# geek-ai/MAgent

Measured on AMD Instinct MI355X. Metric: agent-steps/sec (step+obs) on battle map; bit-exact vs CPU ref, higher is better.
Workload: dtype f32; 1 GPU; battle 1000x1000, 2x400k agents, random placement (C3(i): 2x500k does not fit 996,004 cells), random actions; envs=1, parallelism=replicas x1, gather=none, rccl_ranks=1, io=device-resident (env_*_device C-ABI)

## Files before the change

### magent_amd/csrc/engine.h

```cpp
#pragma once
#include <hip/hip_runtime.h>
#include <stdint.h>

namespace magent_amd {

constexpr int MAXG = 8;
constexpr int REF_SHIFT = 27;
constexpr int REF_MASK = (1 << REF_SHIFT) - 1;
constexpr int OCC_EMPTY = -1;
constexpr int OCC_WALL = -2;
constexpr int OCC_FOOD = -3;

constexpr int PEND_NONE = 0;
constexpr int PEND_MOVE = 1 << 16;
constexpr int PEND_ATTACK = 2 << 16;
constexpr int PEND_TURN = 3 << 16;
constexpr int PEND_ARG = 0xFFFF;

constexpr int OP_KILL = 3, OP_COLLIDE = 6, OP_ATTACK = 7, OP_NULL = 11;

constexpr int RANK_INF = 0x7FFFFFFF;
constexpr unsigned MV_FAIL = 0xFFFFFFFFu, MV_OK = 0xFFFFFFFEu;
constexpr unsigned MV_SILENT = 0xFFFFFFFDu, MV_TAKEN_BIT = 0x80000000u;
__host__ __device__ inline bool mv_taken(unsigned s) { return (s >> 30) == 2u; }
// ... 18 lines not shown
        default: rx = x + ln - 1; ry = y; break;
    }
}
__host__ __device__ inline void real_to_saved(int dir, int wd, int ln, int rx, int ry, int &x, int &y) {
    switch (dir) {
        case DIR_NORTH: x = rx; y = ry; break;
        case DIR_SOUTH: x = rx - wd + 1; y = ry - ln + 1; break;
        case DIR_WEST: x = rx; y = ry - wd + 1; break;
        default: x = rx - ln + 1; y = ry; break;
    }
}

__host__ __device__ inline int ref_pack(int g, int i) { return (g << REF_SHIFT) | i; }
__host__ __device__ inline int ref_group(int r) { return r >> REF_SHIFT; }
__host__ __device__ inline int ref_index(int r) { return r & REF_MASK; }

struct TypeDev {
    float hp, damage, step_recover, kill_supply, kill_reward, dead_penalty, attack_penalty, step_reward;
    float food_supply, eat_ability;
    int attack_in_group;
    int can_absorb;
    int bw, bl;
    int n_move, n_attack;
    int n_turn;
    int move_off, attack_off;
    int attack_bit;
    int view_w, view_h;
    int view_x1, view_y1;
    int mask_off;
};
// ... 89 lines not shown
```

### magent_amd/csrc/engine_batch.hip

```cpp
#include "engine_impl.h"

namespace magent_amd {

bool Env::cycle_eligible(int n_group, float *const *view, float *const *feat, int *first_obs_out) {
    if (!device_ready) fatal("cycle called before reset");
    const int NG = (int)groups.size();
    if (n_group != NG) fatal("env_cycle_many: n_group (%d) differs from the number of groups (%d)", n_group, NG);
    return solo_ok(total_agents()) && !step_pending && !serial_calls_on && observed_groups_ok(view, feat, true, false, first_obs_out);
}

bool Env::observed_groups_ok(float *const *view, float *const *feat, bool goals_differ, bool refuse_acted, int *first_obs_out) const {
    int n_obs = 0, first_obs = -1;
    if (first_obs_out) *first_obs_out = -1;
    for (int g = 0; g < (int)groups.size(); g++) {
        if (refuse_acted && groups[g].acted) return false;
        if (!(view && view[g]) || groups[g].n == 0) continue;
        if (!feat || !feat[g] || (((uintptr_t)view[g]) & 15) || (((uintptr_t)feat[g]) & 15)) return false;
        const HostType &t = *groups[g].type, &t0 = *groups[first_obs < 0 ? g : first_obs].type;
        if (minimap_mode && (t.view.height != t0.view.height || t.view.width != t0.view.width || (goals_differ && t.can_absorb != t0.can_absorb))) return false;
        if (first_obs < 0) first_obs = g;
        n_obs++;
    }
    if (first_obs_out) *first_obs_out = first_obs;
    return n_obs <= RENDER_MULTI_MAX;
// ... 300 lines not shown
    if ((size_t)sa_tiles > asums_cap) {
        grow(arena, d_asums, asums_cap, (size_t)sa_tiles, stream);
        grow(arena, d_wpre, wpre_cap, asums_cap * (SCAN_TILE_HOST / 64), stream);
    }
    step_live_paint = live_paint_now = paint_valid;
    step_pending = true;
    map_warm = false;
    step_kind = StepKind::Pipeline; step_fused_rules = true;
    plain_steps++;
    scratch_for(Scratch::Plain);
    shuffle_buffers(total_n);
    push_rng();
    attack_round = rounds;
    if (rounds >= 4) pairs_two_steps++; else if (rounds >= 2) pairs_one_steps++;
    it.W.live_paint = live_paint_now ? 1 : 0;
    it.PW = plain_view();
    it.ptab = d_ptab; it.gtab = d_gtab; it.ttab = d_ttab;
    it.B = shuffle_bufs(); it.powtab = d_powtab;
    it.sums = d_asums; it.wpre = d_wpre;
    it.R = strike_rules(rule_args.data(), (int)rule_args.size());
    it.seq = ++step_seq;
    it.n_max = total_n;
    alive_valid = true;
    stale_events = true;
    for (auto &g : groups) g.sa_off = -1;
    it.A = ClearArgs{};
    for (int g = 0; g < NG; g++) {
        HostGroup &G = groups[g];
        if (rewards && rewards[g] && G.n > 0) { it.rewards[g] = rewards[g]; it.group_reward[g] = G.group_reward; }
        it.A.sums_off[g] = alive_off[g];
// ... 44 lines not shown
```

### magent_amd/csrc/engine_host.h

```cpp
#pragma once
#include <condition_variable>
#include <functional>
#include <map>
#include <memory>
#include <mutex>
#include <string>
#include <thread>
#include <utility>
#include <vector>

#include "engine.h"
#include "launch.h"
#include "tune.h"

namespace magent_amd {

[[noreturn]] void fatal(const char *fmt, ...);

struct MinStd {
    unsigned long long x = 1;
    void seed(unsigned long s) { x = s % 2147483647ul; if (x == 0) x = 1; }
    unsigned long long operator()() { x = (x * 16807ull) % 2147483647ull; return x; }
    void skip(unsigned n) {
        unsigned long long b = 16807ull, a = x;
// ... 220 lines not shown
    void wait_record(int seq);
    StepRecord *h_rec = nullptr;
    int step_seq = 0;
    int solo_nt_eval = 0;
    unsigned *d_hit = nullptr;
    int2 *d_mvnodes = nullptr; size_t mvnodes_cap = 0;
    void move_nodes();
    bool claim_clean = false;
    bool claim_epochs = false;
    unsigned plain_epoch = 0;
    bool hit_clean = false;
    void scratch_for(Scratch path);
    int plain_steps = 0, plain_slots = 0;
    int pairs_two_steps = 0, pairs_one_steps = 0, claim_refills = 0;
    bool plain_world = false, step_fused_rules = false, ptab_valid = false;
    PlainGroup *d_ptab = nullptr;
    int *d_alive = nullptr; size_t alive_cap = 0;
    int alive_off[MAXG] = {}, alive_n[MAXG] = {};
    bool alive_valid = false;
    bool map_scattered = false;
    long long placed_random = 0, placed_total = 0;
    bool map_warm = false;
    PlainWorld plain_view();
    void plain_arrays(HostGroup &g, size_t n, size_t cap);
    bool stale_events = false;
    RuleArgs *d_rule_args = nullptr; RuleProg *d_rule_progs = nullptr;
    void shuffle_buffers(int n_max);
    void push_rng();
    ShuffleBufs shuffle_bufs() const;
    void attack_rounds_checked(const WorldView &W);
// ... 77 lines not shown
```

### magent_amd/csrc/engine_step.hip

```cpp
#include "engine_impl.h"

namespace magent_amd {

void Env::set_action_device(int g, const int *d_act) {
    if (g < 0 || g >= (int)groups.size()) fatal("invalid group handle in set_action : %d", g);
    use_device();
    HostGroup &G = groups[g];
    bool goals_act = G.type->can_absorb && G.n > 0 && !G.acted && !serial_calls_on;
    if (goals_act) {
        enter();
        int *flag = d_counters + CTR_GOALS_ACT;
        HIP_OK(hipMemsetAsync(flag, 0, sizeof(int), stream));
        launch_any_real_action(stream, d_act, G.n, G.tdev, d_delta, flag);
        int h_flag = 0;
        read_back(&h_flag, flag, sizeof(int));
        goals_act = h_flag != 0;
        static bool told = false;
        if (goals_act && !told) {
            told = true;
            std::fprintf(stderr, "magent-amd: a group of goals (can_absorb) was given actions that move, turn or attack: such steps run the reference's "
                                 "sequential loops on one lane of the device -- exact, about a microsecond per action of the whole world (INTEGRATION.md)\n");
        }
    }
    if (G.acted || serial_calls_on || goals_act) {
// ... 289 lines not shown
    shuffle_buffers(total_n);
    push_rng();
    scratch_for(Scratch::Solo);
    assign_pending_seq(W);
    const SoloStep S = solo_step_args();
    ProfScope p(*this, "step");
    launch_step_solo(stream, W, S);
}

bool Env::single_sync_step(const WorldView &W, int total_n, bool beside) {
    const bool plain = W.plain != 0;
    step_kind = plain ? StepKind::Pipeline : StepKind::Generic;
    if (plain) plain_steps++;
    scratch_for(plain ? Scratch::Plain : Scratch::Other);
    PlainWorld PW{};
    if (plain) PW = plain_view();
    {
        const size_t caps = rank_cap + shuf_cap + sums_cap + powtab_cap;
        const bool rng_here = !rng_on_device;
        shuffle_buffers(total_n);
        push_rng();
        if (rng_here || caps != rank_cap + shuf_cap + sums_cap + powtab_cap) state_epoch++;
    }
    hipStream_t a = beside ? side_stream() : stream;
    {
        ProfScope p(*this, "attack", false, a);
        if (plain) launch_shuffle_draw(a, total_n, d_counters, shuffle_bufs(), d_powtab, step_sa_tiled);
        else launch_shuffle(a, total_n, d_counters, shuffle_bufs(), d_rank, d_hit, (size_t)width * height, d_powtab, step_sa_tiled);
        if (overlap_level == 2 && a != stream) { join_side(); a = stream; }
        attack_round = 0;
        const int pairs = opt_fixed ? opt_attack_pairs : (boost_attack > 0 ? 2 : 1);
        if (plain) { if (pairs >= 2) pairs_two_steps++; else if (pairs == 1) pairs_one_steps++; }
        if (plain) launch_plain_rank(a, W, PW, d_ptab, shuffle_bufs(), d_asums, d_wpre, seq_plan());
        else launch_attack_rank(a, W, d_gtab, d_rank, shuffle_bufs(), false, d_asums, d_wpre, seq_plan());
        for (int r = 0; r < 2 * pairs; r++) {
            const int flag = r == 2 * pairs - 1 ? CTR_OPEN_ATTACK : -1;
            if (plain) launch_plain_eval(a, W, PW, d_ptab, d_gtab, d_ttab, ++attack_round, flag, shuffle_bufs());
            else launch_attack_iter(a, W, d_gtab, d_ttab, ++attack_round, attack_kmax, flag);
        }
        if (pairs == 0) launch_set_counter(a, d_counters, CTR_OPEN_ATTACK, 1, -1);
    }
    join_side();
    if (!plain) { generic_step_tail(W); return false; }
    return plain_step_tail(W, PW);
}

bool Env::plain_step_tail(const WorldView &W, const PlainWorld &PW) {
    const bool fuse = step_fused_rules = !rules_on_host && !stale_events && fused_rules(rule_args.data(), (int)rule_args.size());
// ... 98 lines not shown
}

PlainWorld Env::plain_view() {
    PlainWorld PW{};
    for (size_t g = 0; g < groups.size(); g++) PW.g[g] = groups[g].pl;
    PW.S = plain_slots; PW.kmax = attack_kmax;
    {
        size_t total = 0;
        for (size_t g = 0; g < groups.size(); g++) { alive_off[g] = (int)total; alive_n[g] = groups[g].n; total += (size_t)(groups[g].n + 255) / 256; }
        grow(arena, d_alive, alive_cap, std::max<size_t>(total, 1), stream);
        PW.alive = d_alive;
        for (int g = 0; g < MAXG; g++) PW.alive_off[g] = g < (int)groups.size() ? alive_off[g] : 0;
    }
    PW.epoch = 62 - (int)(plain_epoch % 63u);
    PW.round_base = (int)(plain_epoch * 64u);
    if (!ptab_valid) {
        if (!d_ptab) HIP_OK(dev_malloc(arena, &d_ptab, sizeof(PlainGroup) * MAXG));
        HIP_OK(hipMemcpyAsync(d_ptab, PW.g, sizeof(PlainGroup) * MAXG, hipMemcpyHostToDevice, stream));
        ptab_valid = true;
        state_epoch++;
    }
    return PW;
}

SeqPlan Env::seq_plan() const {
    SeqPlan P{};
    for (int g = 0; g < MAXG; g++) P.off[g] = g < (int)groups.size() ? groups[g].sa_off : -1;
    return P;
}

// ... 181 lines not shown
```

### magent_amd/csrc/launch.h

```cpp
#pragma once
#include "engine.h"

namespace magent_amd {

struct FastDiv {
    unsigned mul, shift, one;
};
inline FastDiv make_fastdiv(unsigned d) {
    FastDiv f{0, 0, 0};
    if (d <= 1) { f.one = 1; return f; }
    unsigned s = 0;
    while ((1ull << s) < d) s++;
    unsigned long long m = ((1ull << 32) * ((1ull << s) - d)) / d + 1;
    f.mul = (unsigned)m;
    f.shift = s - 1;
    return f;
}

struct RenderPlan {
    int spans;
    int steps_per_span;
    int feat_blocks;
    int xcd_chunk;
    int strip_floats;
// ... 84 lines not shown
struct SeqPlan { int off[MAXG]; };
void launch_set_action(hipStream_t s, const WorldView &W, int g, const int *actions, int call_base, int *sums, int *wpre, int tile_off );
void launch_seq_assign(hipStream_t s, const WorldView &W, int g, const int *sums, const int *wpre, int tile_off, bool write_total);
void launch_attack_rank(hipStream_t s, const WorldView &W, const GroupDev *gtab, const int *rank, const ShuffleBufs &B, bool clear_hitbits, const int *sums, const int *wpre,
                        const SeqPlan &P);
void launch_attack_iter(hipStream_t s, const WorldView &W, const GroupDev *gtab, const TypeDev *ttab, int round, int kmax, int flag );
void launch_attack_apply(hipStream_t s, const WorldView &W, const GroupDev *gtab, const TypeDev *ttab, int kmax);
struct PlainGroup { int4 *rec; int *atk; unsigned *hmask; uint2 *hlist; };
struct PlainWorld {
    PlainGroup g[MAXG];
    int S, kmax;
    int *alive;
    int alive_off[MAXG];
    int epoch;
    int round_base;
};
struct StrikeRules {
    int n;
    struct One { int ga, gb, op, rule_no, n_subj; float v[4]; } r[4];
};
StrikeRules strike_rules(const RuleArgs *rules , int n_rules);
bool fused_rules(const RuleArgs *rules, int n);
bool plain_eval_lds_ok(int kmax);
void launch_shuffle_draw(hipStream_t s, int n_max, int *counters, const ShuffleBufs &B, const unsigned *powtab, bool tiled);
void launch_plain_rank(hipStream_t s, const WorldView &W, const PlainWorld &PW, const PlainGroup *ptab, const ShuffleBufs &B, const int *sums,
                       const int *wpre, const SeqPlan &P);
void launch_plain_eval(hipStream_t s, const WorldView &W, const PlainWorld &PW, const PlainGroup *ptab, const GroupDev *gtab, const TypeDev *ttab, int round, int flag,
                       const ShuffleBufs &B);
void launch_plain_tail(hipStream_t s, const WorldView &W, const PlainWorld &PW, const PlainGroup *ptab, const GroupDev *gtab, const TypeDev *ttab,
                       const RuleArgs *rules , int n_rules, StepRecord *rec , int seq);
void launch_food_iter(hipStream_t s, const WorldView &W, const GroupDev *gtab, const TypeDev *ttab, int round, int kmax, int flag);
void launch_attack_events(hipStream_t s, const WorldView &W, int4 *ev);
void launch_move_prep(hipStream_t s, const WorldView &W, const GroupDev *gtab);
void launch_movg_prep(hipStream_t s, const WorldView &W, bool starve);
void launch_turn_prep(hipStream_t s, const WorldView &W);
void launch_turn_sweep(hipStream_t s, const WorldView &W, const GroupDev *gtab, int flag);
void launch_turn_apply(hipStream_t s, const WorldView &W);
void launch_movg_sweep(hipStream_t s, const WorldView &W, const GroupDev *gtab, int flag);
void launch_movg_apply(hipStream_t s, const WorldView &W, const GroupDev *gtab);
void launch_move_apply(hipStream_t s, const WorldView &W, const GroupDev *gtab);
void launch_rule(hipStream_t s, const WorldView &W, const RuleArgs &A);
// ... 28 lines not shown
    const PlainGroup *ptab; const GroupDev *gtab; const TypeDev *ttab;
    ShuffleBufs B; const unsigned *powtab;
    int *sums, *wpre;
    SeqPlan P;
    const int *actions[MAXG]; int call_base[MAXG];
    StrikeRules R;
    StepRecord *rec; int seq;
    int n_max;
    RenderMulti M;
    ClearArgs A;
    MiniArgs Mi; int *counts;
    const int *alive_sums;
    float *rewards[MAXG]; float group_reward[MAXG];
    GroupDev *gtab_out; TypeDev *ttab_out;
    int *newn;
    int pad_[2];
};
struct PipeCtl { const StepRecord *reports_d; StepRecord *reports_h; int *ticket; int *flag_h; int flag_seq; int n_env; };
constexpr int PIPE_REPORT_BYTES = 128;
struct PipeDims { int n_env, max_n, max_total, G, slots, render_blocks, rounds, kmax, sweep, hist_cells; size_t render_lds; };
void launch_pipe_upload(hipStream_t s, const PipeItem *h_items, PipeItem *d_items, int n_env);
void launch_pipe_cycle(hipStream_t s, const PipeItem *d_items, const PipeDims &D, const PipeCtl &C);
bool render_sweep_mini_ok(const WorldView &W, const RenderArgs &R);
size_t render_sweep_lds(int VHW, int C);

#ifndef MAGENT_SCAN_ITEMS
#define MAGENT_SCAN_ITEMS 2
#endif
constexpr int SCAN_ITEMS_HOST = MAGENT_SCAN_ITEMS;
constexpr int SCAN_TILE_HOST = 256 * SCAN_ITEMS_HOST;
constexpr int ATTACK_KMAX_HOST = 32;
// ... 3 lines not shown
```

### magent_amd/csrc/plain_dev.h

```cpp
#pragma once
#include "kernels_dev.h"

namespace magent_amd {

__device__ __forceinline__ void set_action_tile_body(const WorldView &W, int g, const int *actions, int call_base, int *sums, int *wpre, int tile_off) {
    const GroupDev &G = W.grp[g];
    const TypeDev &T = W.type[g];
    const int tile0 = blockIdx.x * SCAN_TILE;
    int act[SCAN_ITEMS], xs[SCAN_ITEMS];
#pragma unroll
    for (int k = 0; k < SCAN_ITEMS; k++) {
        const int i = tile0 + k * SCAN_THREADS + threadIdx.x;
        act[k] = i < G.n ? actions[i] : 0;
        xs[k] = (i < G.n && W.large_map) ? G.x[i] : 0;
    }
    __shared__ int s_w[SCAN_WAVES];
#pragma unroll
    for (int k = 0; k < SCAN_ITEMS; k++) {
        const int i = tile0 + k * SCAN_THREADS + threadIdx.x;
        const bool attack = i < G.n && act[k] >= T.n_move + T.n_turn && act[k] < T.n_move + T.n_turn + T.n_attack;
        const int cnt = __popcll(__ballot(attack));
        if (lane_id() == 0) s_w[k * (SCAN_THREADS / 64) + (threadIdx.x >> 6)] = cnt;
        if (i < G.n) {
            const int a = act[k];
// ... 63 lines not shown
        rec->unsupported = counters[CTR_UNSUPPORTED]; rec->pack_overflow = counters[CTR_PACK_OVERFLOW];
        rec->bad_action = counters[CTR_BAD_ACTION]; rec->hit_overflow = counters[CTR_HIT_OVERFLOW];
        rec->error = 0; rec->rounds_attack = 0; rec->rounds_move = 0; rec->n_marks = 0;
        rec->open_attack = oa; rec->open_move = om;
    }
    if (!open) {
        if (tid < CTR_TRIGGER_END - CTR_TRIGGER) counters[CTR_TRIGGER + tid] = 0;
        if (tid < ROUND_SLOTS) counters[CTR_ROUND_CHANGED + tid] = 0;
        if (tid < ATT_SLOTS) counters[att_slot(tid)] = 0;
        if (tid == 0) counters[CTR_ATTACK] = 0;
    }
    if (mode == REPORT_DEVICE) { if (tid == 0) rec->seq = seq; return; }
    __threadfence_system();
    if (tid == 0) __hip_atomic_store((int *)&rec->seq, seq, __ATOMIC_RELEASE, __HIP_MEMORY_SCOPE_SYSTEM);
}
__device__ __forceinline__ void plain_rank_body(const WorldView &W, const PlainWorld &PW, const PlainGroup *ptab, const ShuffleBufs &B, const int *sums, const int *wpre, const SeqPlan &P) {
    const int A = W.counters[CTR_ATTACK];
    if ((blockIdx.x | blockIdx.y | threadIdx.x) == 0) {
        W.counters[CTR_CHANGED] = 0;
        W.counters[CTR_LAST_A] = A;
        W.counters[CTR_RNG] = (int)rng_skip((unsigned)W.counters[CTR_RNG], (unsigned)A);
    }
    const int g = blockIdx.y;
    const int i = blockIdx.x * blockDim.x + threadIdx.x;
    const GroupDev &G = W.grp[g];
    const TypeDev &T = W.type[g];
    const int n = G.n;
    if ((int)(blockIdx.x * blockDim.x) >= n) return;
    const int pend = i < n ? G.pend[i] : PEND_NONE;
    const bool att = (pend & ~PEND_ARG) == PEND_ATTACK;
    int seq = -1;
    if (A != 0 && P.off[g] >= 0) seq = attack_seq(sums, wpre, P.off[g], i, att);
    if (i >= n) return;
    const bool dead = G.dead[i];
    const int x = G.x[i], y = G.y[i];
    unsigned key = G.key[i];
    int tgt = -1, t = -1;
    if (!dead && att) {
        key = (unsigned)shuffle_chase_pos(seq >= 0 ? seq : (int)key, A, B.j, B.head, B.first, B.link);
        const int k = pend & PEND_ARG;
        const int2 d = W.delta[T.attack_off + k];
        const int tx = x + d.x, ty = y + d.y;
        if (tx >= 0 && tx < W.w && ty >= 0 && ty < W.h) {
            const int o = W.occ[ty * W.w + tx];
            if (o >= 0 && (T.attack_in_group || ref_group(o) != g)) {
                tgt = o;
                const PlainGroup TG = ptab[ref_group(o)];
                const int slot = T.attack_bit + k;
                glob(TG.hlist)[(size_t)ref_index(o) * PW.S + slot] = make_uint2(key, (unsigned)ref_pack(g, i));
                atomicOr(&glob(TG.hmask)[ref_index(o)], 1u << slot);
            }
        }
    } else if (!dead && (pend & ~PEND_ARG) == PEND_MOVE) {
        const int2 d = W.delta[T.move_off + (pend & PEND_ARG)];
        const int nx = x + d.x, ny = y + d.y;
        if ((d.x | d.y) != 0 && nx >= 0 && ny >= 0 && nx + 1 < W.w && ny + 1 < W.h) t = ny * W.w + nx;
    }
    PW.g[g].rec[i] = make_int4((int)key, dead ? -1 : RANK_INF, t, (int)MV_FAIL_SAME);
    PW.g[g].atk[i] = tgt;
    if (!(T.step_recover > 0)) G.mv[i] = __float_as_uint(G.hp[i]);
}

__device__ __forceinline__ void plain_eval_body(const WorldView &W, const PlainWorld &PW, const PlainGroup *ptab, const GroupDev *gtab, const TypeDev *ttab, int round, int flag,
                                                int *shuf_head, int *shuf_first) {
    const int A = W.counters[CTR_ATTACK];
    const int prev_changed = W.counters[CTR_ROUND_CHANGED + ((round - 1) & (ROUND_SLOTS - 1))];
    if (A == 0) return;
    if (round == 1)
        for (int k = (blockIdx.y * gridDim.x + blockIdx.x) * blockDim.x + threadIdx.x; k < A; k += gridDim.x * gridDim.y * blockDim.x) {
            shuf_head[k] = 0; shuf_first[k] = 0;
        }
    if (round > 1 && prev_changed == 0) return;
    extern __shared__ unsigned s_hit[];
    const int NT = blockDim.x, tid = threadIdx.x;
    unsigned *s_rank = s_hit;
// ... 18 lines not shown
    sort_hits(s_rank, s_ref, NT, tid, nh);
    float hp = G.hp[i];
    int dr = RANK_INF;
    for (int k = 0; k < nh; k++) {
        const unsigned r = s_rank[k * NT + tid];
        const int a = s_ref[k * NT + tid];
        const int adr = glob(ptab[ref_group(a)].rec)[ref_index(a)].y;
        if ((unsigned)adr >= r) {
            hp -= ttab[ref_group(a)].damage;
            if (hp < 0.0f) { dr = (int)r; break; }
        }
    }
    G.mv[i] = __float_as_uint(hp);
    if (dr != dr_cur) {
        PW.g[g].rec[i].y = dr;
        const int reader = PW.g[g].atk[i];
        if (reader >= 0) glob(gtab[ref_group(reader)].drank_b)[ref_index(reader)] = PW.round_base + round;
        if (flag >= 0) W.counters[flag] = 1;
        W.counters[CTR_ROUND_CHANGED + (round & (ROUND_SLOTS - 1))] = 1;
    }
}

__device__ __forceinline__ void strike_body(const WorldView &W, const PlainWorld &PW, const PlainGroup *ptab, const GroupDev *gtab, const TypeDev *ttab, const StrikeRules &R) {
    const int g = blockIdx.y, i = blockIdx.x * blockDim.x + threadIdx.x;
    const GroupDev &G = W.grp[g];
    const TypeDev &T = W.type[g];
    if ((int)(blockIdx.x * blockDim.x) >= G.n) return;
    const int il = i < G.n ? i : G.n - 1;
    const int pend = G.pend[il];
    const int4 me = PW.g[g].rec[il];
    const float hp0 = G.hp[il], nr0 = G.next_reward[il];
    const bool dead0 = G.dead[il];
    if (attack_open(W)) return;
    const bool attacked = W.counters[CTR_ATTACK] != 0;
    bool died = false, alive = false;
    unsigned trig = 0;
    if (i < G.n) {
        if (pend != PEND_NONE) G.last_action[i] = pend_action(pend, T);
        bool dead = dead0;
        float hp = hp0;
        const unsigned hp_before = __float_as_uint(hp);
        float nr = nr0;
        const unsigned nr_before = __float_as_uint(nr);
        int last_op = OP_NULL, op_obj = -1;
        if (attacked && !dead) {
            if (PW.g[g].hmask[i]) {
                PW.g[g].hmask[i] = 0u;
                hp = __uint_as_float(G.mv[i]);
            }
            if ((pend & ~PEND_ARG) == PEND_ATTACK) {
                const unsigned my_rank = (unsigned)me.x;
                const int tgt = PW.g[g].atk[i];
                int tgt_dr = RANK_INF;
                if (tgt >= 0) tgt_dr = glob(ptab[ref_group(tgt)].rec)[ref_index(tgt)].y;
                if ((unsigned)me.y >= my_rank) {
                    float own;
                    if (tgt < 0 || (unsigned)tgt_dr < my_rank) own = T.attack_penalty;
                    else {
                        float reward = 0.0f;
                        if ((unsigned)tgt_dr == my_rank) { last_op = OP_KILL; reward = ttab[ref_group(tgt)].kill_reward; }
                        else last_op = OP_ATTACK;
                        op_obj = tgt;
                        G.last_op[i] = (unsigned char)last_op; G.op_obj[i] = tgt;
                        own = reward + T.attack_penalty;
                    }
                    nr += own;
                }
// ... 9 lines not shown
        }
        if (__float_as_uint(hp) != hp_before) G.hp[i] = hp;
        if (died) G.dead[i] = 1;
        alive = !dead;
        for (int k = 0; k < R.n; k++) {
            if (R.r[k].ga != g) continue;
            if (op_obj >= 0 && ref_group(op_obj) == R.r[k].gb && last_op == R.r[k].op) {
                trig |= 1u << k;
                for (int q = 0; q < R.r[k].n_subj; q++) nr += R.r[k].v[q];
            }
        }
        if (__float_as_uint(nr) != nr_before) G.next_reward[i] = nr;
        if (!dead && me.z >= 0) {
            const int c = me.z;
            const unsigned key = (unsigned)me.x;
            int o = W.occ[c];
            bool ok = o == OCC_EMPTY;
            if (o == OCC_WALL) PW.g[g].rec[i].z = -1;
            if (o >= 0) {
                const int4 oc = glob(ptab[ref_group(o)].rec)[ref_index(o)];
                const float orec = ttab[ref_group(o)].step_recover;
                bool gone = attacked && oc.y != RANK_INF;
                if (!gone && !(orec > 0)) gone = __uint_as_float(glob(gtab[ref_group(o)].mv)[ref_index(o)]) - (-orec) < 0.0f;
                if (gone) { ok = true; o = OCC_EMPTY; }
                else ok = oc.z >= 0 && (unsigned)oc.x < key;
            }
            PW.g[g].atk[i] = o;
            if (ok) atomicMin(&W.claim[c], claim_word(PW.epoch, key, ref_pack(g, i)));
        }
        if (died) PW.g[g].rec[i].w = (int)MV_DIED;
        else if (__float_as_uint(hp) != hp_before) PW.g[g].rec[i].w = (int)MV_FAIL;
    }
    int wtot;
    wave_rank(died, wtot);
    if (wtot && lane_id() == 0) atomicAdd(&W.counters[dead_slot(g, blockIdx.x % DEAD_SLOTS)], wtot);
    for (int k = 0; k < R.n; k++)
        if (__ballot((trig >> k) & 1u) && lane_id() == 0) W.counters[CTR_TRIGGER + R.r[k].rule_no] = 1;
    __shared__ int s_alive[4];
    const int alive_w = __popcll(__ballot(alive));
    if (lane_id() == 0) s_alive[threadIdx.x >> 6] = alive_w;
    __syncthreads();
    if (threadIdx.x == 0 && (int)(blockIdx.x * blockDim.x) < G.n) PW.alive[PW.alive_off[g] + blockIdx.x] = s_alive[0] + s_alive[1] + s_alive[2] + s_alive[3];
// ... 16 lines not shown
        if (ra.z < 0) return MV_FAIL;
        const unsigned long long cl = glob(W.claim)[ra.z];
        if (!claim_live(cl, PW.epoch) || claim_ref(cl) != a) return MV_FAIL;
        const int o = plain_atk(PW, W.G, ref_group(a))[ref_index(a)];
        if (o == OCC_EMPTY) return MV_OK;
        a = o;
        ra = plain_rec(PW, W.G, ref_group(a))[ref_index(a)];
    }
}
__device__ __forceinline__ void plain_commit_body(const WorldView &W, const PlainWorld &PW, StepRecord *rec, int seq, int report_mode = REPORT_HOST) {
    if (rec && (blockIdx.x | blockIdx.y) == 0 && threadIdx.x < 64) step_report_body(glob(W.counters), glob(rec), seq, W.G, report_mode);
    const int g = blockIdx.y, i = blockIdx.x * blockDim.x + threadIdx.x;
    const GroupDev G = glob_group(W.grp[g]);
    if (i >= G.n) return;
    const int4 me = glob(PW.g[g].rec)[i];
    const int o = glob(PW.g[g].atk)[i];
    const int px = G.x[i], py = G.y[i];
    if (attack_open(W)) return;
    const int self = ref_pack(g, i), old = py * W.w + px, c = me.z;
    const bool died = (unsigned)me.w == MV_DIED;
    const bool mover = c >= 0 && !died;
    const bool alive = me.y != -1 && !died;
    const bool chain = mover && o >= 0;
    const unsigned long long cl_c = glob(W.claim)[mover ? c : 0];
    const bool old_now = died || (mover && !chain);
    unsigned long long cl_old = glob(W.claim)[old_now ? old : 0];
    const int4 ro = plain_rec(PW, W.G, chain ? ref_group(o) : g)[chain ? ref_index(o) : i];
    const unsigned s_o = chain ? plain_leaves(W, PW, o, ro) : MV_OK;
    const bool winner = mover && claim_live(cl_c, PW.epoch) && claim_ref(cl_c) == self;
    const bool ok = winner && s_o == MV_OK;
    if (ok && !old_now) cl_old = glob(W.claim)[old];
    int cell = old;
    if (ok) {
        if (!claim_live(cl_old, PW.epoch)) { glob(W.occ)[old] = OCC_EMPTY; if (W.live_paint) vc_store(W, old, OCC_EMPTY, 0u); }
        glob(W.occ)[c] = self;
        const int ny = c / W.w;
        G.x[i] = c - ny * W.w; G.y[i] = ny;
        cell = c;
    } else if (mover) {
        int blocker;
        if (o == OCC_EMPTY) blocker = claim_ref(cl_c);
        else blocker = (s_o == MV_OK && (unsigned)ro.x < (unsigned)me.x) ? claim_ref(cl_c) : o;
        G.last_op[i] = OP_COLLIDE;
        G.op_obj[i] = blocker;
    } else if (died && !claim_live(cl_old, PW.epoch)) { glob(W.occ)[old] = OCC_EMPTY; if (W.live_paint) vc_store(W, old, OCC_EMPTY, 0u); }
    G.pend[i] = PEND_NONE;
    if (W.live_paint && alive && (ok || (unsigned)me.w == MV_FAIL))
        vc_store(W, cell, g, __float_as_uint(__fdiv_rn(G.hp[i], W.type[g].hp)));
}
__device__ __forceinline__ void clear_compact_body(const WorldView &W, const ClearArgs &A, int mode, const int *sums, const MiniArgs &M, int *counts,
                                                   float *reward_out = nullptr, float group_reward = 0.0f) {
    extern __shared__ int s_hist[];
    const int g = blockIdx.y;
    const GroupDev &G = W.grp[g];
    if ((int)(blockIdx.x * SCAN_TILE) >= G.n) return;
    const float step_reward = W.type[g].step_reward;
// ... 46 lines not shown
```

### magent_amd/csrc/step.hip

```cpp
#include "plain_dev.h"

namespace magent_amd {

__global__ void k_set_counter(int *counters, int index, int value, int unless_index) {
    if (threadIdx.x == 0 && !(unless_index >= 0 && counters[unless_index])) counters[index] = value;
}
__global__ void k_step_reset(int *counters) {
    if (threadIdx.x == 0) counters[CTR_ATTACK] = 0;
    for (int k = CTR_TRIGGER + threadIdx.x; k < CTR_TRIGGER_END; k += blockDim.x) counters[k] = 0;
    for (int k = threadIdx.x; k < ROUND_SLOTS; k += blockDim.x) counters[CTR_ROUND_CHANGED + k] = 0;
    for (int k = threadIdx.x; k < ATT_SLOTS; k += blockDim.x) counters[att_slot(k)] = 0;
}
__global__ void __launch_bounds__(64) k_step_report(int *counters, StepRecord *rec, int seq, int NG, int mode) { step_report_body(counters, rec, seq, NG, mode); }
static int report_mode() { return REPORT_HOST; }
__global__ void k_set_rng(int *counters, unsigned x) { if (threadIdx.x == 0) counters[CTR_RNG] = (int)x; }

__global__ void __launch_bounds__(256) k_fill32_gated(WorldView W, unsigned *p, unsigned v, size_t n) {
    if (attack_open(W)) return;
    for (size_t i = blockIdx.x * (size_t)blockDim.x + threadIdx.x; i < n; i += (size_t)gridDim.x * blockDim.x) p[i] = v;
}

__global__ void __launch_bounds__(256) k_fill32(unsigned *p, unsigned v, size_t n) {
    for (size_t i = blockIdx.x * (size_t)blockDim.x + threadIdx.x; i < n; i += (size_t)gridDim.x * blockDim.x) p[i] = v;
}
// ... 150 lines not shown
__global__ void __launch_bounds__(256) k_move_init(WorldView W) {
    if (attack_open(W)) return;
    const int g = blockIdx.y, i = blockIdx.x * blockDim.x + threadIdx.x;
    if (i < W.grp[g].n) move_init_body(W, g, i);
}
__global__ void __launch_bounds__(256) k_move_commit(WorldView W, const GroupDev *gtab) {
    if (step_open(W)) return;
    const int g = blockIdx.y, i = blockIdx.x * blockDim.x + threadIdx.x;
    if (i >= W.grp[g].n) return;
    move_commit_body(W, gtab, g, i);
    if (W.live_paint) repaint_body(W, W.grp[g], W.type[g], g, i);
}

__global__ void __launch_bounds__(256) k_plain_rank(WorldView W, PlainWorld PW, const PlainGroup *ptab, ShuffleBufs B, const int *sums, const int *wpre, SeqPlan P) {
    plain_rank_body(W, PW, ptab, B, sums, wpre, P);
}
__global__ void __launch_bounds__(256) k_plain_eval(WorldView W, PlainWorld PW, const PlainGroup *ptab, const GroupDev *gtab, const TypeDev *ttab, int round, int flag,
                                                   int *shuf_head, int *shuf_first) {
    plain_eval_body(W, PW, ptab, gtab, ttab, round, flag, shuf_head, shuf_first);
}
__global__ void __launch_bounds__(256) k_strike(WorldView W, PlainWorld PW, const PlainGroup *ptab, const GroupDev *gtab, const TypeDev *ttab, StrikeRules R) {
    strike_body(W, PW, ptab, gtab, ttab, R);
}
__global__ void __launch_bounds__(256) k_plain_commit(WorldView W, PlainWorld PW, StepRecord *rec, int seq, int report_mode) {
    plain_commit_body(W, PW, rec, seq, report_mode);
}
__global__ void __launch_bounds__(256) k_movg_prep(WorldView W, unsigned *wanted, int starve) {
    if (attack_open(W)) return;
    if ((blockIdx.x | blockIdx.y | threadIdx.x) == 0) W.counters[CTR_CHANGED] = 0;
    movg_prep_body(W, blockIdx.y, blockIdx.x * blockDim.x + threadIdx.x, wanted, blockIdx.x % DEAD_SLOTS, starve != 0);
// ... 422 lines not shown
StrikeRules strike_rules(const RuleArgs *rules, int n_rules) {
    StrikeRules R{};
    if (rules) {
        R.n = n_rules;
        for (int k = 0; k < n_rules; k++) {
            R.r[k].ga = rules[k].ga; R.r[k].gb = rules[k].gb; R.r[k].op = rules[k].op; R.r[k].rule_no = rules[k].rule_no; R.r[k].n_subj = rules[k].n_subj;
            for (int q = 0; q < 4; q++) R.r[k].v[q] = rules[k].v_subj[q];
        }
    }
    return R;
}
void launch_plain_rank(hipStream_t s, const WorldView &W, const PlainWorld &PW, const PlainGroup *ptab, const ShuffleBufs &B, const int *sums,
                       const int *wpre, const SeqPlan &P) {
    hipLaunchKernelGGL(k_plain_rank, grid_all(W, 256), dim3(256), 0, s, W, PW, ptab, B, sums, wpre, P);
}
size_t plain_eval_lds(int kmax) { return (size_t)kmax * 256 * 8; }
bool plain_eval_lds_ok(int kmax) {
    if (plain_eval_lds(kmax) <= (48u << 10)) return true;
    return hipFuncSetAttribute(reinterpret_cast<const void *>(k_plain_eval), hipFuncAttributeMaxDynamicSharedMemorySize, (int)plain_eval_lds(kmax)) == hipSuccess;
}
void launch_plain_eval(hipStream_t s, const WorldView &W, const PlainWorld &PW, const PlainGroup *ptab, const GroupDev *gtab, const TypeDev *ttab, int round, int flag,
                       const ShuffleBufs &B) {
    hipLaunchKernelGGL(k_plain_eval, grid_all(W, 256), dim3(256), plain_eval_lds(PW.kmax), s, W, PW, ptab, gtab, ttab, round, flag, B.head, B.first);
}
void launch_shuffle_draw(hipStream_t s, int n_max, int *counters, const ShuffleBufs &B, const unsigned *powtab, bool tiled) {
    hipLaunchKernelGGL(k_shuffle_draw, dim3((n_max + 255) / 256), dim3(256), 0, s, counters, B.j, B.head, B.first, B.link, (unsigned *)nullptr, (size_t)0, powtab, tiled ? 1 : 0);
}
void launch_plain_tail(hipStream_t s, const WorldView &W, const PlainWorld &PW, const PlainGroup *ptab, const GroupDev *gtab, const TypeDev *ttab,
                       const RuleArgs *rules, int n_rules, StepRecord *rec, int seq) {
    const StrikeRules R = strike_rules(rules, n_rules);
// ... 95 lines not shown
```

### magent_amd/csrc/tune.h

```cpp
#pragma once
#include <cstdio>
#include <cstdlib>
#include <cstring>

namespace magent_amd {

inline void tune_refuse_removed_variables() {
    static const char *const removed[][2] = {
        {"MAGENT_CHECKED_STEP", "checked_step"}, {"MAGENT_HOST_SHUFFLE", "host_shuffle"}, {"MAGENT_OPT_ATTACK_PAIRS", "attack_pairs"},
        {"MAGENT_OPT_MOVE_BATCHES", "move_batches"}, {"MAGENT_SOLO_STEP", "solo_step"}, {"MAGENT_SOLO_MAX", "solo_max"},
        {"MAGENT_SCAN_SOLO_MAX", "scan_solo_max"}, {"MAGENT_OVERLAP", "overlap"}, {"MAGENT_FOLD_MINIMAP", "fold_minimap"},
        {"MAGENT_RENDER_FAST", "render"}, {"MAGENT_RENDER_SWEEP", "render_sweep"}, {"MAGENT_RENDER_SU", "render_su"},
        {"MAGENT_RENDER_DEPTH", "render_depth"}, {"MAGENT_ATT_THREADS", "att_threads"}, {"MAGENT_POLICY_GRID", "policy_grid"},
        {"MAGENT_BATCH_CYCLE", "batch_cycle"}, {"MAGENT_HIP_POLICY", nullptr}, {"MAGENT_FEAT_SEPARATE", nullptr}, {"MAGENT_RENDER_NT", nullptr},
        {"MAGENT_RENDER_SPAN", nullptr}, {"MAGENT_RENDER_UNROLL", nullptr}, {"MAGENT_RENDER_PAD", nullptr}, {"MAGENT_RENDER_XCD", nullptr}};
    for (const auto &r : removed)
        if (std::getenv(r[0])) {
            if (r[1]) std::fprintf(stderr, "magent-amd FATAL: the environment variable %s is no longer read: use MAGENT_TUNE=%s=... (magent_amd/csrc/tune.h)\n", r[0], r[1]);
            else std::fprintf(stderr, "magent-amd FATAL: the environment variable %s is no longer read and has no successor: the knob was removed (magent_amd/csrc/tune.h)\n", r[0]);
            std::abort();
        }
}

inline int tune(const char *key, int dflt) {
    static const bool legacy_checked = (tune_refuse_removed_variables(), true);
    (void)legacy_checked;
    static const char *const known[] = {"checked_step", "host_shuffle", "attack_pairs", "move_batches", "solo_step", "solo_max", "batch_solo_max", "scan_solo_max", "overlap",
                                        "fold_minimap", "render", "render_sweep", "render_su", "render_depth", "att_threads", "policy_grid", "policy_stamps",
                                        "batch_cycle", "early_report", "touch_map", "batch_pipe", "batch_pipe_min", "pipe_sweep", "pipe_span", "pipe_own"};
    const char *s = std::getenv("MAGENT_TUNE");
    if (!s || !*s) return dflt;
    static bool checked = false;
    if (!checked) {
        checked = true;
        for (const char *p = s; *p;) {
            const char *e = std::strchr(p, ',');
            const size_t len = e ? (size_t)(e - p) : std::strlen(p);
            const char *eq = (const char *)std::memchr(p, '=', len);
            bool ok = false;
            if (eq)
                for (const char *k : known) ok |= std::strlen(k) == (size_t)(eq - p) && !std::strncmp(k, p, (size_t)(eq - p));
            if (!ok && len) { std::fprintf(stderr, "magent-amd FATAL: MAGENT_TUNE: unknown entry \"%.*s\" (see magent_amd/csrc/tune.h)\n", (int)len, p); std::abort(); }
            if (!e) break;
            p = e + 1;
// ... 16 lines not shown
```

Baseline: 728.3 million agent-steps/s.

## Fuse shuffle draw with plain prep and split rank chase into lean kernel

Replaces the separate shuffle-draw and plain-rank launches with a combined open kernel that draws the shuffle and prepares per-agent records in one grid. A following chase kernel resolves shuffle ranks only for attackers with a real target. Movers look up the target cell once in prep and reuse it in eval, and commit marks blocked moves so they skip claim reads. The aim is fewer launches, less redundant chase work and fewer occupancy/claim reads, at the cost of extra state bits, an extra kernel and more branching.

```diff
diff --git a/magent_amd/csrc/engine.h b/magent_amd/csrc/engine.h
--- a/magent_amd/csrc/engine.h
+++ b/magent_amd/csrc/engine.h
@@ -56,6 +56,8 @@
 __host__ __device__ inline int ref_pack(int g, int i) { return (g << REF_SHIFT) | i; }
 __host__ __device__ inline int ref_group(int r) { return r >> REF_SHIFT; }
 __host__ __device__ inline int ref_index(int r) { return r & REF_MASK; }
+constexpr int ATK_BLOCKED = 1 << 30;
+static_assert((((MAXG - 1) << REF_SHIFT) | REF_MASK) < ATK_BLOCKED, "bit 30 of a packed agent reference must be spare");
 
 struct TypeDev {
     float hp, damage, step_recover, kill_supply, kill_reward, dead_penalty, attack_penalty, step_reward;
diff --git a/magent_amd/csrc/engine_batch.hip b/magent_amd/csrc/engine_batch.hip
--- a/magent_amd/csrc/engine_batch.hip
+++ b/magent_amd/csrc/engine_batch.hip
@@ -338,6 +338,7 @@
     attack_round = rounds;
     if (rounds >= 4) pairs_two_steps++; else if (rounds >= 2) pairs_one_steps++;
     it.W.live_paint = live_paint_now ? 1 : 0;
+    step_plain_open = false;
     it.PW = plain_view();
     it.ptab = d_ptab; it.gtab = d_gtab; it.ttab = d_ttab;
     it.B = shuffle_bufs(); it.powtab = d_powtab;
diff --git a/magent_amd/csrc/engine_host.h b/magent_amd/csrc/engine_host.h
--- a/magent_amd/csrc/engine_host.h
+++ b/magent_amd/csrc/engine_host.h
@@ -258,6 +258,7 @@
     int plain_steps = 0, plain_slots = 0;
     int pairs_two_steps = 0, pairs_one_steps = 0, claim_refills = 0;
     bool plain_world = false, step_fused_rules = false, ptab_valid = false;
+    bool step_plain_open = false;
     PlainGroup *d_ptab = nullptr;
     int *d_alive = nullptr; size_t alive_cap = 0;
     int alive_off[MAXG] = {}, alive_n[MAXG] = {};
diff --git a/magent_amd/csrc/engine_step.hip b/magent_amd/csrc/engine_step.hip
--- a/magent_amd/csrc/engine_step.hip
+++ b/magent_amd/csrc/engine_step.hip
@@ -327,6 +327,8 @@
     if (plain) plain_steps++;
     scratch_for(plain ? Scratch::Plain : Scratch::Other);
     PlainWorld PW{};
+    static const bool open_wanted = tune("plain_open", 1) != 0;
+    step_plain_open = plain && open_wanted;
     if (plain) PW = plain_view();
     {
         const size_t caps = rank_cap + shuf_cap + sums_cap + powtab_cap;
@@ -338,13 +340,15 @@
     hipStream_t a = beside ? side_stream() : stream;
     {
         ProfScope p(*this, "attack", false, a);
-        if (plain) launch_shuffle_draw(a, total_n, d_counters, shuffle_bufs(), d_powtab, step_sa_tiled);
+        if (plain && step_plain_open) launch_plain_open(a, total_n, W, PW, shuffle_bufs(), d_powtab, step_sa_tiled, d_asums, d_wpre, seq_plan());
+        else if (plain) launch_shuffle_draw(a, total_n, d_counters, shuffle_bufs(), d_powtab, step_sa_tiled);
         else launch_shuffle(a, total_n, d_counters, shuffle_bufs(), d_rank, d_hit, (size_t)width * height, d_powtab, step_sa_tiled);
         if (overlap_level == 2 && a != stream) { join_side(); a = stream; }
         attack_round = 0;
         const int pairs = opt_fixed ? opt_attack_pairs : (boost_attack > 0 ? 2 : 1);
         if (plain) { if (pairs >= 2) pairs_two_steps++; else if (pairs == 1) pairs_one_steps++; }
-        if (plain) launch_plain_rank(a, W, PW, d_ptab, shuffle_bufs(), d_asums, d_wpre, seq_plan());
+        if (plain && step_plain_open) launch_plain_chase(a, W, PW, d_ptab, shuffle_bufs());
+        else if (plain) launch_plain_rank(a, W, PW, d_ptab, shuffle_bufs(), d_asums, d_wpre, seq_plan());
         else launch_attack_rank(a, W, d_gtab, d_rank, shuffle_bufs(), false, d_asums, d_wpre, seq_plan());
         for (int r = 0; r < 2 * pairs; r++) {
             const int flag = r == 2 * pairs - 1 ? CTR_OPEN_ATTACK : -1;
@@ -473,6 +477,8 @@
     }
     PW.epoch = 62 - (int)(plain_epoch % 63u);
     PW.round_base = (int)(plain_epoch * 64u);
+    static const int lean = (tune("lean_chase", 1) ? LEAN_CHASE : 0) | (tune("lean_commit", 1) ? LEAN_COMMIT : 0);
+    PW.lean = lean | (step_plain_open ? LEAN_OPEN : 0);
     if (!ptab_valid) {
         if (!d_ptab) HIP_OK(dev_malloc(arena, &d_ptab, sizeof(PlainGroup) * MAXG));
         HIP_OK(hipMemcpyAsync(d_ptab, PW.g, sizeof(PlainGroup) * MAXG, hipMemcpyHostToDevice, stream));
diff --git a/magent_amd/csrc/launch.h b/magent_amd/csrc/launch.h
--- a/magent_amd/csrc/launch.h
+++ b/magent_amd/csrc/launch.h
@@ -122,7 +122,10 @@
     int alive_off[MAXG];
     int epoch;
     int round_base;
-};
+    int lean;
+};
+constexpr int LEAN_CHASE = 1, LEAN_COMMIT = 2, LEAN_OPEN = 4;
+struct OpenPlan { int n_draw; int first[MAXG + 1]; };
 struct StrikeRules {
     int n;
     struct One { int ga, gb, op, rule_no, n_subj; float v[4]; } r[4];
@@ -133,6 +136,9 @@
 void launch_shuffle_draw(hipStream_t s, int n_max, int *counters, const ShuffleBufs &B, const unsigned *powtab, bool tiled);
 void launch_plain_rank(hipStream_t s, const WorldView &W, const PlainWorld &PW, const PlainGroup *ptab, const ShuffleBufs &B, const int *sums,
                        const int *wpre, const SeqPlan &P);
+void launch_plain_open(hipStream_t s, int n_max, const WorldView &W, const PlainWorld &PW, const ShuffleBufs &B, const unsigned *powtab, bool tiled, const int *sums,
+                       const int *wpre, const SeqPlan &P);
+void launch_plain_chase(hipStream_t s, const WorldView &W, const PlainWorld &PW, const PlainGroup *ptab, const ShuffleBufs &B);
 void launch_plain_eval(hipStream_t s, const WorldView &W, const PlainWorld &PW, const PlainGroup *ptab, const GroupDev *gtab, const TypeDev *ttab, int round, int flag,
                        const ShuffleBufs &B);
 void launch_plain_tail(hipStream_t s, const WorldView &W, const PlainWorld &PW, const PlainGroup *ptab, const GroupDev *gtab, const TypeDev *ttab,
@@ -191,7 +197,6 @@
     float *rewards[MAXG]; float group_reward[MAXG];
     GroupDev *gtab_out; TypeDev *ttab_out;
     int *newn;
-    int pad_[2];
 };
 struct PipeCtl { const StepRecord *reports_d; StepRecord *reports_h; int *ticket; int *flag_h; int flag_seq; int n_env; };
 constexpr int PIPE_REPORT_BYTES = 128;
diff --git a/magent_amd/csrc/plain_dev.h b/magent_amd/csrc/plain_dev.h
--- a/magent_amd/csrc/plain_dev.h
+++ b/magent_amd/csrc/plain_dev.h
@@ -101,51 +101,83 @@
     __threadfence_system();
     if (tid == 0) __hip_atomic_store((int *)&rec->seq, seq, __ATOMIC_RELEASE, __HIP_MEMORY_SCOPE_SYSTEM);
 }
-__device__ __forceinline__ void plain_rank_body(const WorldView &W, const PlainWorld &PW, const PlainGroup *ptab, const ShuffleBufs &B, const int *sums, const int *wpre, const SeqPlan &P) {
-    const int A = W.counters[CTR_ATTACK];
-    if ((blockIdx.x | blockIdx.y | threadIdx.x) == 0) {
-        W.counters[CTR_CHANGED] = 0;
-        W.counters[CTR_LAST_A] = A;
-        W.counters[CTR_RNG] = (int)rng_skip((unsigned)W.counters[CTR_RNG], (unsigned)A);
-    }
-    const int g = blockIdx.y;
-    const int i = blockIdx.x * blockDim.x + threadIdx.x;
+struct PlainPrep { int entry, tgt, slot; bool chases; int4 rec; };
+__device__ __forceinline__ PlainPrep plain_prep_body(const WorldView &W, const PlainWorld &PW, const int *sums, const int *wpre, const SeqPlan &P, int g, int tile, bool with_a, bool chase_follows) {
+    PlainPrep R{-1, -1, 0, false, make_int4(0, 0, 0, 0)};
+    const int i = tile * 256 + threadIdx.x;
     const GroupDev &G = W.grp[g];
     const TypeDev &T = W.type[g];
     const int n = G.n;
-    if ((int)(blockIdx.x * blockDim.x) >= n) return;
+    if (tile * 256 >= n) return R;
     const int pend = i < n ? G.pend[i] : PEND_NONE;
     const bool att = (pend & ~PEND_ARG) == PEND_ATTACK;
     int seq = -1;
-    if (A != 0 && P.off[g] >= 0) seq = attack_seq(sums, wpre, P.off[g], i, att);
-    if (i >= n) return;
+    if (P.off[g] >= 0 && (!with_a || W.counters[CTR_ATTACK] != 0)) seq = attack_seq(sums, wpre, P.off[g], i, att);
+    if (i >= n) return R;
     const bool dead = G.dead[i];
     const int x = G.x[i], y = G.y[i];
     unsigned key = G.key[i];
     int tgt = -1, t = -1;
     if (!dead && att) {
-        key = (unsigned)shuffle_chase_pos(seq >= 0 ? seq : (int)key, A, B.j, B.head, B.first, B.link);
+        if (seq >= 0) key = (unsigned)seq;
         const int k = pend & PEND_ARG;
         const int2 d = W.delta[T.attack_off + k];
         const int tx = x + d.x, ty = y + d.y;
         if (tx >= 0 && tx < W.w && ty >= 0 && ty < W.h) {
             const int o = W.occ[ty * W.w + tx];
-            if (o >= 0 && (T.attack_in_group || ref_group(o) != g)) {
-                tgt = o;
-                const PlainGroup TG = ptab[ref_group(o)];
-                const int slot = T.attack_bit + k;
-                glob(TG.hlist)[(size_t)ref_index(o) * PW.S + slot] = make_uint2(key, (unsigned)ref_pack(g, i));
-                atomicOr(&glob(TG.hmask)[ref_index(o)], 1u << slot);
-            }
-        }
+            if (o >= 0 && (T.attack_in_group || ref_group(o) != g)) tgt = o;
+        }
+        R.entry = (int)key; R.tgt = tgt; R.slot = T.attack_bit + k; R.chases = tgt >= 0 || !(PW.lean & LEAN_CHASE);
     } else if (!dead && (pend & ~PEND_ARG) == PEND_MOVE) {
         const int2 d = W.delta[T.move_off + (pend & PEND_ARG)];
         const int nx = x + d.x, ny = y + d.y;
         if ((d.x | d.y) != 0 && nx >= 0 && ny >= 0 && nx + 1 < W.w && ny + 1 < W.h) t = ny * W.w + nx;
-    }
-    PW.g[g].rec[i] = make_int4((int)key, dead ? -1 : RANK_INF, t, (int)MV_FAIL_SAME);
+        if ((PW.lean & LEAN_OPEN) && t >= 0) {
+            tgt = W.occ[t];
+            if (tgt == OCC_WALL) { t = -1; tgt = -1; }
+        }
+    }
+    R.rec = make_int4((int)key, dead ? -1 : RANK_INF, t, (int)MV_FAIL_SAME);
+    if (!(chase_follows && R.chases)) PW.g[g].rec[i] = R.rec;
     PW.g[g].atk[i] = tgt;
     if (!(T.step_recover > 0)) G.mv[i] = __float_as_uint(G.hp[i]);
+    return R;
+}
+__device__ __forceinline__ void plain_chase_head(const WorldView &W) {
+    const int A = W.counters[CTR_ATTACK];
+    W.counters[CTR_CHANGED] = 0;
+    W.counters[CTR_LAST_A] = A;
+    W.counters[CTR_RNG] = (int)rng_skip((unsigned)W.counters[CTR_RNG], (unsigned)A);
+}
+__device__ __forceinline__ void plain_chase_body(const WorldView &W, const PlainWorld &PW, const PlainGroup *ptab, const ShuffleBufs &B, int g, int i, int entry, int tgt, int slot,
+                                                 const int4 *whole = nullptr) {
+    const int A = W.counters[CTR_ATTACK];
+    const unsigned rank = (unsigned)shuffle_chase_pos(entry, A, B.j, B.head, B.first, B.link);
+    if (whole) PW.g[g].rec[i] = make_int4((int)rank, whole->y, whole->z, whole->w);
+    else PW.g[g].rec[i].x = (int)rank;
+    if (tgt >= 0) {
+        const PlainGroup TG = ptab[ref_group(tgt)];
+        glob(TG.hlist)[(size_t)ref_index(tgt) * PW.S + slot] = make_uint2(rank, (unsigned)ref_pack(g, i));
+        atomicOr(&glob(TG.hmask)[ref_index(tgt)], 1u << slot);
+    }
+}
+__device__ __forceinline__ void plain_rank_body(const WorldView &W, const PlainWorld &PW, const PlainGroup *ptab, const ShuffleBufs &B, const int *sums, const int *wpre, const SeqPlan &P) {
+    if ((blockIdx.x | blockIdx.y | threadIdx.x) == 0) plain_chase_head(W);
+    const PlainPrep R = plain_prep_body(W, PW, sums, wpre, P, blockIdx.y, blockIdx.x, true, true);
+    if (R.chases) plain_chase_body(W, PW, ptab, B, blockIdx.y, blockIdx.x * 256 + threadIdx.x, R.entry, R.tgt, R.slot, &R.rec);
+}
+__device__ __forceinline__ void plain_chase_launch_body(const WorldView &W, const PlainWorld &PW, const PlainGroup *ptab, const ShuffleBufs &B) {
+    if ((blockIdx.x | blockIdx.y | threadIdx.x) == 0) plain_chase_head(W);
+    const int g = blockIdx.y, i = blockIdx.x * blockDim.x + threadIdx.x;
+    const GroupDev &G = W.grp[g];
+    if (i >= G.n) return;
+    const int pend = G.pend[i];
+    const int tgt = PW.g[g].atk[i];
+    if ((pend & ~PEND_ARG) != PEND_ATTACK) return;
+    if (tgt < 0 && (PW.lean & LEAN_CHASE)) return;
+    const int4 me = PW.g[g].rec[i];
+    if (me.y == -1) return;
+    plain_chase_body(W, PW, ptab, B, g, i, me.x, tgt, W.type[g].attack_bit + (pend & PEND_ARG));
 }
 
 __device__ __forceinline__ void plain_eval_body(const WorldView &W, const PlainWorld &PW, const PlainGroup *ptab, const GroupDev *gtab, const TypeDev *ttab, int round, int flag,
@@ -194,7 +226,7 @@
     G.mv[i] = __float_as_uint(hp);
     if (dr != dr_cur) {
         PW.g[g].rec[i].y = dr;
-        const int reader = PW.g[g].atk[i];
+        const int reader = (G.pend[i] & ~PEND_ARG) == PEND_ATTACK ? PW.g[g].atk[i] : -1;
         if (reader >= 0) glob(gtab[ref_group(reader)].drank_b)[ref_index(reader)] = PW.round_base + round;
         if (flag >= 0) W.counters[flag] = 1;
         W.counters[CTR_ROUND_CHANGED + (round & (ROUND_SLOTS - 1))] = 1;
@@ -211,6 +243,9 @@
     const int4 me = PW.g[g].rec[il];
     const float hp0 = G.hp[il], nr0 = G.next_reward[il];
     const bool dead0 = G.dead[il];
+    const bool att0 = (pend & ~PEND_ARG) == PEND_ATTACK;
+    const bool looked = (PW.lean & LEAN_OPEN) != 0;
+    const int atk0 = (att0 || looked) ? PW.g[g].atk[il] : -1;
     if (attack_open(W)) return;
     const bool attacked = W.counters[CTR_ATTACK] != 0;
     bool died = false, alive = false;
@@ -228,9 +263,9 @@
                 PW.g[g].hmask[i] = 0u;
                 hp = __uint_as_float(G.mv[i]);
             }
-            if ((pend & ~PEND_ARG) == PEND_ATTACK) {
+            if (att0) {
                 const unsigned my_rank = (unsigned)me.x;
-                const int tgt = PW.g[g].atk[i];
+                const int tgt = atk0;
                 int tgt_dr = RANK_INF;
                 if (tgt >= 0) tgt_dr = glob(ptab[ref_group(tgt)].rec)[ref_index(tgt)].y;
                 if ((unsigned)me.y >= my_rank) {
@@ -270,7 +305,7 @@
         if (!dead && me.z >= 0) {
             const int c = me.z;
             const unsigned key = (unsigned)me.x;
-            int o = W.occ[c];
+            int o = looked ? atk0 : W.occ[c];
             bool ok = o == OCC_EMPTY;
             if (o == OCC_WALL) PW.g[g].rec[i].z = -1;
             if (o >= 0) {
@@ -281,7 +316,8 @@
                 if (gone) { ok = true; o = OCC_EMPTY; }
                 else ok = oc.z >= 0 && (unsigned)oc.x < key;
             }
-            PW.g[g].atk[i] = o;
+            if (!ok && o >= 0 && (PW.lean & LEAN_COMMIT)) o |= ATK_BLOCKED;
+            if (!looked || o != atk0) PW.g[g].atk[i] = o;
             if (ok) atomicMin(&W.claim[c], claim_word(PW.epoch, key, ref_pack(g, i)));
         }
         if (died) PW.g[g].rec[i].w = (int)MV_DIED;
@@ -328,20 +364,22 @@
     const GroupDev G = glob_group(W.grp[g]);
     if (i >= G.n) return;
     const int4 me = glob(PW.g[g].rec)[i];
-    const int o = glob(PW.g[g].atk)[i];
+    const int o_word = glob(PW.g[g].atk)[i];
     const int px = G.x[i], py = G.y[i];
     if (attack_open(W)) return;
     const int self = ref_pack(g, i), old = py * W.w + px, c = me.z;
     const bool died = (unsigned)me.w == MV_DIED;
     const bool mover = c >= 0 && !died;
     const bool alive = me.y != -1 && !died;
-    const bool chain = mover && o >= 0;
-    const unsigned long long cl_c = glob(W.claim)[mover ? c : 0];
-    const bool old_now = died || (mover && !chain);
+    const bool blocked = mover && o_word >= 0 && (o_word & ATK_BLOCKED) != 0;
+    const int o = blocked ? o_word & ~ATK_BLOCKED : o_word;
+    const bool chain = mover && o >= 0 && !blocked;
+    const unsigned long long cl_c = glob(W.claim)[mover && !blocked ? c : 0];
+    const bool old_now = died || (mover && !chain && !blocked);
     unsigned long long cl_old = glob(W.claim)[old_now ? old : 0];
     const int4 ro = plain_rec(PW, W.G, chain ? ref_group(o) : g)[chain ? ref_index(o) : i];
     const unsigned s_o = chain ? plain_leaves(W, PW, o, ro) : MV_OK;
-    const bool winner = mover && claim_live(cl_c, PW.epoch) && claim_ref(cl_c) == self;
+    const bool winner = mover && !blocked && claim_live(cl_c, PW.epoch) && claim_ref(cl_c) == self;
     const bool ok = winner && s_o == MV_OK;
     if (ok && !old_now) cl_old = glob(W.claim)[old];
     int cell = old;
@@ -353,7 +391,8 @@
         cell = c;
     } else if (mover) {
         int blocker;
-        if (o == OCC_EMPTY) blocker = claim_ref(cl_c);
+        if (blocked) blocker = o;
+        else if (o == OCC_EMPTY) blocker = claim_ref(cl_c);
         else blocker = (s_o == MV_OK && (unsigned)ro.x < (unsigned)me.x) ? claim_ref(cl_c) : o;
         G.last_op[i] = OP_COLLIDE;
         G.op_obj[i] = blocker;
diff --git a/magent_amd/csrc/step.hip b/magent_amd/csrc/step.hip
--- a/magent_amd/csrc/step.hip
+++ b/magent_amd/csrc/step.hip
@@ -188,6 +188,19 @@
 
 __global__ void __launch_bounds__(256) k_plain_rank(WorldView W, PlainWorld PW, const PlainGroup *ptab, ShuffleBufs B, const int *sums, const int *wpre, SeqPlan P) {
     plain_rank_body(W, PW, ptab, B, sums, wpre, P);
+}
+__global__ void __launch_bounds__(256) k_plain_open(WorldView W, PlainWorld PW, ShuffleBufs B, const unsigned *powtab, int tiled, const int *sums, const int *wpre, SeqPlan P,
+                                                    OpenPlan O) {
+    if ((int)blockIdx.x < O.n_draw) { shuffle_draw_launch_body(W.counters, B.j, B.head, B.first, B.link, nullptr, 0, powtab, tiled); return; }
+    const int b = blockIdx.x - O.n_draw;
+    int g = 0;
+#pragma unroll
+    for (int k = 1; k < MAXG; k++) if (k < W.G && b >= O.first[k]) g = k;
+    g = __builtin_amdgcn_readfirstlane(g);
+    plain_prep_body(W, PW, sums, wpre, P, g, b - O.first[g], false, false);
+}
+__global__ void __launch_bounds__(256) k_plain_chase(WorldView W, PlainWorld PW, const PlainGroup *ptab, ShuffleBufs B) {
+    plain_chase_launch_body(W, PW, ptab, B);
 }
 __global__ void __launch_bounds__(256) k_plain_eval(WorldView W, PlainWorld PW, const PlainGroup *ptab, const GroupDev *gtab, const TypeDev *ttab, int round, int flag,
                                                    int *shuf_head, int *shuf_first) {
@@ -640,6 +653,16 @@
                        const int *wpre, const SeqPlan &P) {
     hipLaunchKernelGGL(k_plain_rank, grid_all(W, 256), dim3(256), 0, s, W, PW, ptab, B, sums, wpre, P);
 }
+void launch_plain_open(hipStream_t s, int n_max, const WorldView &W, const PlainWorld &PW, const ShuffleBufs &B, const unsigned *powtab, bool tiled, const int *sums,
+                       const int *wpre, const SeqPlan &P) {
+    OpenPlan O{};
+    O.n_draw = (n_max + 255) / 256;
+    for (int g = 0; g < MAXG; g++) O.first[g + 1] = O.first[g] + (g < W.G ? (W.grp[g].n + 255) / 256 : 0);
+    hipLaunchKernelGGL(k_plain_open, dim3(O.n_draw + O.first[MAXG]), dim3(256), 0, s, W, PW, B, powtab, tiled ? 1 : 0, sums, wpre, P, O);
+}
+void launch_plain_chase(hipStream_t s, const WorldView &W, const PlainWorld &PW, const PlainGroup *ptab, const ShuffleBufs &B) {
+    hipLaunchKernelGGL(k_plain_chase, grid_all(W, 256), dim3(256), 0, s, W, PW, ptab, B);
+}
 size_t plain_eval_lds(int kmax) { return (size_t)kmax * 256 * 8; }
 bool plain_eval_lds_ok(int kmax) {
     if (plain_eval_lds(kmax) <= (48u << 10)) return true;
diff --git a/magent_amd/csrc/tune.h b/magent_amd/csrc/tune.h
--- a/magent_amd/csrc/tune.h
+++ b/magent_amd/csrc/tune.h
@@ -27,7 +27,8 @@
     (void)legacy_checked;
     static const char *const known[] = {"checked_step", "host_shuffle", "attack_pairs", "move_batches", "solo_step", "solo_max", "batch_solo_max", "scan_solo_max", "overlap",
                                         "fold_minimap", "render", "render_sweep", "render_su", "render_depth", "att_threads", "policy_grid", "policy_stamps",
-                                        "batch_cycle", "early_report", "touch_map", "batch_pipe", "batch_pipe_min", "pipe_sweep", "pipe_span", "pipe_own"};
+                                        "batch_cycle", "early_report", "touch_map", "batch_pipe", "batch_pipe_min", "pipe_sweep", "pipe_span", "pipe_own",
+                                        "lean_chase", "lean_commit", "plain_open"};
     const char *s = std::getenv("MAGENT_TUNE");
     if (!s || !*s) return dflt;
     static bool checked = false;
```

Measured after the change: 730.5 million agent-steps/s (median of 6 runs). No clear change (+0.3%).
